# zz990099/foundationpose_cpp

Measured on AMD Instinct MI355X. Metric: pose-hypotheses/sec (Register N=252, 640x480), higher is better.
Workload: dtype f16; 1 GPU; Register N=252 hypotheses, 640x480 refine_itr=1, frame resident in HBM; mesh=synthetic ellipsoid V=2562 F=5120, 512x512 texture, weights=synthetic (seed 7), precision=f16 storage / f32 accumulate (the reference's TensorRT --fp16), parallelism=single GPU, collective=none

## Files before the change

foundationpose_cpp_amd/csrc/fp_geometry.hip:

```cpp

#include "fp_internal.h"
#include <cstdlib>

namespace fp {

#define CR_SUBPIXEL_LOG2 4
#define CR_MAXVIEWPORT_LOG2 11
#define CR_DEPTH_MIN (2200u << 3)
#define CR_DEPTH_MAX (0xFFFFFFFFu - (2200u << 3))

static constexpr int CROP = FP_CROP_HW;

struct K9 { float k[9]; };

__device__ __forceinline__ float clampf(float f, float a, float b) { return fmaxf(a, fminf(f, b)); }

template <bool FMAD> __device__ __forceinline__ float mad(float a, float b, float c) { return FMAD ? fmaf(a, b, c) : a * b + c; }
template <bool FMAD> __device__ __forceinline__ float dot3(float a0, float b0, float a1, float b1, float a2, float b2) {
  return mad<FMAD>(a2, b2, mad<FMAD>(a1, b1, a0 * b0));
}
template <bool FMAD> __device__ __forceinline__ float diffprod(float a, float b, float c, float d) {
  return FMAD ? fmaf(a, b, -(c * d)) : a * b - c * d;
}

// ... 378 lines not shown
    }
    if (!culled) {
      out = TRI_ROWS_ALL;
      if ((v0.w >= fabsf(v0.z)) & (v1.w >= fabsf(v1.z)) & (v2.w >= fabsf(v2.z))) {
        const float vs = (float)(CROP << (CR_SUBPIXEL_LOG2 - 1));
        const float rw0 = 1.0f / v0.w, rw1 = 1.0f / v1.w, rw2 = 1.0f / v2.w;
        const int ax = f32_to_s32_sat(v0.x * rw0 * vs), ay = f32_to_s32_sat(v0.y * rw0 * vs);
        const int bx_ = f32_to_s32_sat(v1.x * rw1 * vs), by_ = f32_to_s32_sat(v1.y * rw1 * vs);
        const int cx = f32_to_s32_sat(v2.x * rw2 * vs), cy = f32_to_s32_sat(v2.y * rw2 * vs);
        const int loxy = min(imin3(ax, bx_, cx), imin3(ay, by_, cy));
        const int hixy = max(imax3(ax, bx_, cx), imax3(ay, by_, cy));
        const int aabbLimit = (1 << (CR_MAXVIEWPORT_LOG2 + CR_SUBPIXEL_LOG2)) - 1;
        if (loxy >= -32768 && hixy <= 32767 && hixy - loxy <= aabbLimit) {
          const int area = (bx_ - ax) * (cy - ay) - (by_ - ay) * (cx - ax);
          const int bx = (CROP - 1) << (CR_SUBPIXEL_LOG2 - 1);
          const int px0 = max((imin3(ax, bx_, cx) + bx + 15) >> 4, 0), px1 = min((imax3(ax, bx_, cx) + bx) >> 4, CROP - 1);
          const int py0 = max((imin3(ay, by_, cy) + bx + 15) >> 4, 0), py1 = min((imax3(ay, by_, cy) + bx) >> 4, CROP - 1);
          out = (area == 0 || px0 > px1 || py0 > py1) ? TRI_ROWS_EMPTY : ((unsigned)py0 | ((unsigned)py1 << 16));
        }
      }
    }
  }
  return out;
}
__global__ __launch_bounds__(256) void tri_rows_kernel(const int32_t *__restrict__ faces, int F, int V, const float4 *__restrict__ clip_all,
                                                       unsigned *__restrict__ rows_all) {
  const int f = blockIdx.x * 256 + threadIdx.x, n = blockIdx.y;
  if (f >= F) return;
  const float4 *clip = clip_all + (size_t)n * V;
  unsigned out = TRI_ROWS_EMPTY;
  const int i0 = faces[f * 3], i1 = faces[f * 3 + 1], i2 = faces[f * 3 + 2];
  if ((unsigned)i0 < (unsigned)V && (unsigned)i1 < (unsigned)V && (unsigned)i2 < (unsigned)V) out = tri_rows_of(clip[i0], clip[i1], clip[i2]);
  rows_all[(size_t)n * F + f] = out;
}
void launch_tri_rows(hipStream_t s, const DeviceMesh &m, int N, const float4 *clip, unsigned *rows) {
  if (m.F <= 0 || N <= 0) return;
  hipLaunchKernelGGL(tri_rows_kernel, dim3((m.F + 255) / 256, N), dim3(256), 0, s, m.faces, m.F, m.V, clip, rows);
}
constexpr int TRI_LIST = 8192;

template <int MODE, int STRIP_ROWS, int NT, bool FMAD, bool VCOL = false>
__global__ __launch_bounds__(NT) void raster_shade_kernel(
    const int32_t *__restrict__ faces, int F, int V, const float *__restrict__ uvs, const uint8_t *__restrict__ tex,
    int TH, int TW, float downscale, const PoseRec *__restrict__ recs, const float4 *__restrict__ clip_all,
    const float4 *__restrict__ attr_all, void *__restrict__ out_all, int32_t *__restrict__ tri_id_dbg,
    float *__restrict__ rast_dbg, const unsigned *__restrict__ tri_rows_all, const uint32_t *__restrict__ vcol = nullptr) {
  extern __shared__ __attribute__((aligned(16))) unsigned char smem[];
  unsigned long long *zbuf = reinterpret_cast<unsigned long long *>(smem);
  const int strip = blockIdx.x, n = blockIdx.y, tid = threadIdx.x;
  const int row0 = strip * STRIP_ROWS;
  const float4 *clip = clip_all + (size_t)n * V;
  const float4 *attr = attr_all + (size_t)n * V;

  const unsigned long long clear_key = ((unsigned long long)CR_DEPTH_MAX << 32) | 0xFFFFFFFFull;
  for (int i = tid; i < STRIP_ROWS * CROP; i += NT) zbuf[i] = clear_key;
  __syncthreads();

  auto process = [&](int f, const float4 &v0, const float4 &v1, const float4 &v2) {
    if ((v0.w < fabsf(v0.x)) | (v0.w < fabsf(v0.y)) | (v0.w < fabsf(v0.z))) {
      if (((v0.w < +v0.x) & (v1.w < +v1.x) & (v2.w < +v2.x)) | ((v0.w < -v0.x) & (v1.w < -v1.x) & (v2.w < -v2.x)) |
          ((v0.w < +v0.y) & (v1.w < +v1.y) & (v2.w < +v2.y)) | ((v0.w < -v0.y) & (v1.w < -v1.y) & (v2.w < -v2.y)) |
          ((v0.w < +v0.z) & (v1.w < +v1.z) & (v2.w < +v2.z)) | ((v0.w < -v0.z) & (v1.w < -v1.z) & (v2.w < -v2.z)))
        return;
    }
    bool fast = false;
    if ((v0.w >= fabsf(v0.z)) & (v1.w >= fabsf(v1.z)) & (v2.w >= fabsf(v2.z))) {
      const float vs = (float)(CROP << (CR_SUBPIXEL_LOG2 - 1));
      float rw0 = 1.0f / v0.w, rw1 = 1.0f / v1.w, rw2 = 1.0f / v2.w;
      int ax = f32_to_s32_sat(v0.x * rw0 * vs), ay = f32_to_s32_sat(v0.y * rw0 * vs);
      int bx_ = f32_to_s32_sat(v1.x * rw1 * vs), by_ = f32_to_s32_sat(v1.y * rw1 * vs);
      int cx = f32_to_s32_sat(v2.x * rw2 * vs), cy = f32_to_s32_sat(v2.y * rw2 * vs);
      int loxy = min(imin3(ax, bx_, cx), imin3(ay, by_, cy));
      int hixy = max(imax3(ax, bx_, cx), imax3(ay, by_, cy));
      const int aabbLimit = (1 << (CR_MAXVIEWPORT_LOG2 + CR_SUBPIXEL_LOG2)) - 1;
      fast = (loxy >= -32768 && hixy <= 32767 && hixy - loxy <= aabbLimit);
    }
    if (fast) raster_one<STRIP_ROWS>(v0, v1, v2, (unsigned)(f + 1), row0, zbuf);
    else raster_clipped<STRIP_ROWS, FMAD>(v0, v1, v2, (unsigned)(f + 1), row0, zbuf);
  };
  struct Tri { int i0, i1, i2; };
  auto load_idx = [&](int f) {
    Tri t{-1, -1, -1};
    if (f < F) { t.i0 = faces[f * 3]; t.i1 = faces[f * 3 + 1]; t.i2 = faces[f * 3 + 2]; }
    return t;
  };
  auto valid = [&](const Tri &t) { return (unsigned)t.i0 < (unsigned)V && (unsigned)t.i1 < (unsigned)V && (unsigned)t.i2 < (unsigned)V; };
  const float4 zero4 = make_float4(0.f, 0.f, 0.f, 0.f);
  if (tri_rows_all) {
    static_assert(TRI_LIST >= 8 * NT, "a slab of 4 NT triangles must fit behind the flush threshold");
    unsigned *list = reinterpret_cast<unsigned *>(zbuf + STRIP_ROWS * CROP);
    unsigned *count = list + TRI_LIST;
    const unsigned *tri_rows = tri_rows_all + (size_t)n * F;
    const unsigned row_last = (unsigned)(row0 + STRIP_ROWS - 1);
    if (tid == 0) *count = 0u;
    __syncthreads();
    auto flush = [&]() {
      const int nl = (int)*count;
      auto entry = [&](int k) { return k < nl ? load_idx((int)list[k]) : Tri{-1, -1, -1}; };
      Tri cur = entry(tid), nxt = entry(tid + NT);
      bool ok = valid(cur);
      float4 v0 = ok ? clip[cur.i0] : zero4, v1 = ok ? clip[cur.i1] : zero4, v2 = ok ? clip[cur.i2] : zero4;
      for (int k = tid; k < nl; k += NT) {
        const bool okn = valid(nxt);
        const float4 w0 = okn ? clip[nxt.i0] : zero4, w1 = okn ? clip[nxt.i1] : zero4, w2 = okn ? clip[nxt.i2] : zero4;
        const Tri nn = entry(k + 2 * NT);
        if (ok) process((int)list[k], v0, v1, v2);
        v0 = w0; v1 = w1; v2 = w2; ok = okn; nxt = nn;
      }
    };
    auto load_slab = [&](int base, unsigned (&r)[4]) {
#pragma unroll
      for (int u = 0; u < 4; u++) {
        const int f = base + u * NT + tid;
        r[u] = f < F ? tri_rows[f] : TRI_ROWS_EMPTY;
      }
    };
    unsigned r[4], rn[4];
    load_slab(0, r);
    for (int base = 0; base < F; base += 4 * NT) {
      load_slab(base + 4 * NT, rn);
#pragma unroll
      for (int u = 0; u < 4; u++)
        if ((r[u] & 0xffffu) <= row_last && (r[u] >> 16) >= (unsigned)row0) list[atomicAdd(count, 1u)] = (unsigned)(base + u * NT + tid);
      __syncthreads();
      const bool full = *count > (unsigned)(TRI_LIST - 4 * NT) && base + 4 * NT < F;
      __syncthreads();
      if (full) {
        flush();
        __syncthreads();
        if (tid == 0) *count = 0u;
        __syncthreads();
      }
#pragma unroll
      for (int u = 0; u < 4; u++) r[u] = rn[u];
    }
    flush();
  } else {
    Tri cur = load_idx(tid), nxt = load_idx(tid + NT);
    bool ok = valid(cur);
    float4 v0 = ok ? clip[cur.i0] : zero4, v1 = ok ? clip[cur.i1] : zero4, v2 = ok ? clip[cur.i2] : zero4;
    for (int f = tid; f < F; f += NT) {
      const bool okn = valid(nxt);
      const float4 w0 = okn ? clip[nxt.i0] : zero4, w1 = okn ? clip[nxt.i1] : zero4, w2 = okn ? clip[nxt.i2] : zero4;
      const Tri nn = load_idx(f + 2 * NT);
      if (ok) process(f, v0, v1, v2);
      v0 = w0; v1 = w1; v2 = w2; ok = okn; nxt = nn;
    }
  }
  __syncthreads();

  const PoseRec &rec = recs[n];
  const float tpx = rec.pose[12], tpy = rec.pose[13], tpz = rec.pose[14];
  const float xs = 2.f / (float)CROP, xo = 1.f / (float)CROP - 1.f;
  for (int i = tid; i < STRIP_ROWS * CROP; i += NT) {
    int ly = i / CROP, px = i - ly * CROP, py = row0 + ly;
    unsigned color = ~(unsigned)(zbuf[i] & 0xFFFFFFFFull);
    int triIdx = (int)color - 1;
    float b0 = 0, b1 = 0, zw = 0, idf = 0;
    float xyz0 = 0, xyz1 = 0, xyz2 = 0, uu = 0, vv = 0, dif = 0;
    float vc[3] = {0, 0, 0};
    if (triIdx >= 0 && triIdx < F) {
      int vi0 = faces[triIdx * 3], vi1 = faces[triIdx * 3 + 1], vi2 = faces[triIdx * 3 + 2];
      float4 p0 = clip[vi0], p1 = clip[vi1], p2 = clip[vi2];
      float fx = mad<FMAD>(xs, (float)px, xo), fy = mad<FMAD>(xs, (float)py, xo);
      float p0x = mad<FMAD>(-fx, p0.w, p0.x), p0y = mad<FMAD>(-fy, p0.w, p0.y);
      float p1x = mad<FMAD>(-fx, p1.w, p1.x), p1y = mad<FMAD>(-fy, p1.w, p1.y);
      float p2x = mad<FMAD>(-fx, p2.w, p2.x), p2y = mad<FMAD>(-fy, p2.w, p2.y);
      float a0 = diffprod<FMAD>(p1x, p2y, p1y, p2x), a1 = diffprod<FMAD>(p2x, p0y, p2y, p0x), a2 = diffprod<FMAD>(p0x, p1y, p0y, p1x);
      float iw = 1.f / (a0 + a1 + a2);
      b0 = a0 * iw; b1 = a1 * iw;
      float z = dot3<FMAD>(p0.z, a0, p1.z, a1, p2.z, a2), w = dot3<FMAD>(p0.w, a0, p1.w, a1, p2.w, a2);
      zw = z / w;
      b0 = clampf(b0, 0.f, 1.f); b1 = clampf(b1, 0.f, 1.f);
      if (b0 != b0) b0 = 0.f;
      if (b1 != b1) b1 = 0.f;
      zw = fmaxf(fminf(zw, 1.f), -1.f);
      idf = (float)(triIdx + 1);
      float b2 = 1.f - b0 - b1;
      float4 q0 = attr[vi0], q1 = attr[vi1], q2 = attr[vi2];
      xyz0 = dot3<FMAD>(b0, q0.x, b1, q1.x, b2, q2.x);
      xyz1 = dot3<FMAD>(b0, q0.y, b1, q1.y, b2, q2.y);
      xyz2 = dot3<FMAD>(b0, q0.z, b1, q1.z, b2, q2.z);
      dif = dot3<FMAD>(b0, q0.w, b1, q1.w, b2, q2.w);
      if constexpr (VCOL) {
        const uint32_t c0 = vcol[vi0], c1 = vcol[vi1], c2 = vcol[vi2];
        const float sc = 1.0f / 255.0f;
#pragma unroll
        for (int c = 0; c < 3; c++)
          vc[c] = dot3<FMAD>(b0, (float)((c0 >> (8 * c)) & 255u) * sc, b1, (float)((c1 >> (8 * c)) & 255u) * sc, b2,
                             (float)((c2 >> (8 * c)) & 255u) * sc);
      } else {
        uu = dot3<FMAD>(b0, uvs[vi0 * 2], b1, uvs[vi1 * 2], b2, uvs[vi2 * 2]);
        vv = dot3<FMAD>(b0, uvs[vi0 * 2 + 1], b1, uvs[vi1 * 2 + 1], b2, uvs[vi2 * 2 + 1]);
      }
    }
    if (tri_id_dbg) tri_id_dbg[((size_t)n * CROP + py) * CROP + px] = (int)color;
    if (rast_dbg) {
      float *ro = rast_dbg + (((size_t)n * CROP + py) * CROP + px) * 4;
      ro[0] = b0; ro[1] = b1; ro[2] = zw; ro[3] = idf;
    }
    float o[6];
    float fg = clampf(idf, 0, 1);
    if (VCOL && fg > 0.0f) {
      const float shade = mad<FMAD>(dif, 0.5f, 0.8f);
      for (int c = 0; c < 3; c++) o[c] = clampf(vc[c] * shade * fg, 0.0f, 1.0f);
    } else if (!VCOL && fg > 0.0f) {
      float u = uu - floorf(uu), v = vv - floorf(vv);
      u = mad<FMAD>(u, (float)TW, -0.5f); v = mad<FMAD>(v, (float)TH, -0.5f);
      int iu0 = (int)floorf(u), iv0 = (int)floorf(v);
      int iu1 = iu0 + 1, iv1 = iv0 + 1;
      u -= (float)iu0; v -= (float)iv0;
      if (iu0 < 0) iu0 += TW;
      if (iv0 < 0) iv0 += TH;
      if (iu1 >= TW) iu1 -= TW;
      if (iv1 >= TH) iv1 -= TH;
      const float sc = 1.0f / 255.0f;
      const uint8_t *t00 = tex + (iu0 + TW * iv0) * 3, *t10 = tex + (iu1 + TW * iv0) * 3;
      const uint8_t *t01 = tex + (iu0 + TW * iv1) * 3, *t11 = tex + (iu1 + TW * iv1) * 3;
      float shade = mad<FMAD>(dif, 0.5f, 0.8f);
      for (int c = 0; c < 3; c++) {
        float a00 = (float)t00[c] * sc, a10 = (float)t10[c] * sc, a01 = (float)t01[c] * sc, a11 = (float)t11[c] * sc;
        float top = mad<FMAD>(u, a10 - a00, a00), bot = mad<FMAD>(u, a11 - a01, a01);
        float rgb = mad<FMAD>(v, bot - top, top);
        float q = rgb * shade * fg;
        o[c] = clampf(clampf(q, 0, 1), 0.0f, 1.0f);
      }
    } else {
      o[0] = o[1] = o[2] = 0.0f;
    }
    {
      bool invalid = xyz2 < FP_MIN_DEPTH;
      float q0 = (xyz0 - tpx) / downscale, q1 = (xyz1 - tpy) / downscale, q2 = (xyz2 - tpz) / downscale;
      o[3] = (fabsf(q0) > FP_MAX_DEPTH || invalid) ? 0.0f : q0;
      o[4] = (fabsf(q1) > FP_MAX_DEPTH || invalid) ? 0.0f : q1;
      o[5] = (fabsf(q2) > FP_MAX_DEPTH || invalid) ? 0.0f : q2;
    }
    size_t opix = ((size_t)n * CROP + (CROP - 1 - py)) * CROP + px;
    if (MODE == OUT_F32X6) {
      float *d = reinterpret_cast<float *>(out_all) + opix * 6;
      float2 *d2 = reinterpret_cast<float2 *>(d);
      d2[0] = make_float2(o[0], o[1]); d2[1] = make_float2(o[2], o[3]); d2[2] = make_float2(o[4], o[5]);
    } else {
      reinterpret_cast<uint4 *>(out_all)[s2d_index((size_t)n, CROP - 1 - py, px)] = pack6<MODE>(o);
    }
  }
}

static thread_local const unsigned *t_tri_rows = nullptr;
static size_t tri_list_lds() { return t_tri_rows ? (size_t)TRI_LIST * 4 + 16 : 0; }

#ifdef FP_TEST_HOOKS
static int g_tri_rows_tall = 0;
void set_tri_rows_tall(int v) { g_tri_rows_tall = v; }
#else
static constexpr int g_tri_rows_tall = 0;
#endif
#ifdef FP_TEST_HOOKS
static int g_strip_threads = 0;
void set_raster_strip_threads(int t) { g_strip_threads = t; }
#else
static constexpr int g_strip_threads = 0;
#endif

template <int MODE, int STRIP_ROWS, bool FMAD, bool VCOL>
static void launch_raster_shade_t(hipStream_t s, const DeviceMesh &m, const PoseRec *recs, int N, const float4 *clip,
                                  const float4 *attr, void *out, int32_t *tri_id_dbg, float *rast_dbg) {
  size_t lds = (size_t)STRIP_ROWS * CROP * sizeof(unsigned long long) + tri_list_lds();
  dim3 grid(CROP / STRIP_ROWS, N), block(256);
  float downscale = m.diameter / 2;
  if constexpr (STRIP_ROWS == 8 && MODE != OUT_F32X6) if (!tri_id_dbg && !rast_dbg && g_strip_threads != 256) {
    if (g_strip_threads == 1024 || (g_strip_threads == 0 && N <= 25)) {
      hipLaunchKernelGGL((raster_shade_kernel<MODE, STRIP_ROWS, 1024, FMAD, VCOL>), grid, dim3(1024), lds, s, m.faces, m.F, m.V, m.uvs,
                         m.tex, m.TH, m.TW, downscale, recs, clip, attr, out, tri_id_dbg, rast_dbg, t_tri_rows, m.vcol);
      return;
    }
    if (g_strip_threads == 512 || (g_strip_threads == 0 && N < 48)) {
      hipLaunchKernelGGL((raster_shade_kernel<MODE, STRIP_ROWS, 512, FMAD, VCOL>), grid, dim3(512), lds, s, m.faces, m.F, m.V, m.uvs,
                         m.tex, m.TH, m.TW, downscale, recs, clip, attr, out, tri_id_dbg, rast_dbg, t_tri_rows, m.vcol);
      return;
    }
  }
  if constexpr (STRIP_ROWS >= 40) {
    static PerDeviceOnce attr_once;
    attr_once.run([] {
      (void)hipFuncSetAttribute((const void *)raster_shade_kernel<MODE, STRIP_ROWS, 256, FMAD, VCOL>, hipFuncAttributeMaxDynamicSharedMemorySize,
                                (int)((size_t)STRIP_ROWS * CROP * sizeof(unsigned long long) + (size_t)TRI_LIST * 4 + 16));
    });
  }
  hipLaunchKernelGGL((raster_shade_kernel<MODE, STRIP_ROWS, 256, FMAD, VCOL>), grid, block, lds, s, m.faces, m.F, m.V, m.uvs, m.tex,
                     m.TH, m.TW, downscale, recs, clip, attr, out, tri_id_dbg, rast_dbg, t_tri_rows, m.vcol);
}

#ifdef FP_TEST_HOOKS
static int g_strip_rows_override = 0;
void set_raster_strip_rows(int r) { g_strip_rows_override = r; }
#else
static constexpr int g_strip_rows_override = 0;
#endif

template <int MODE, int STRIP_ROWS, bool FMAD, bool VCOL>
static void launch_raster_tall(hipStream_t s, const DeviceMesh &m, const PoseRec *recs, int N, const float4 *clip,
                               const float4 *attr, void *out) {
  const size_t lds_max = (size_t)STRIP_ROWS * CROP * sizeof(unsigned long long) + (size_t)TRI_LIST * 4 + 16;
  size_t lds = (size_t)STRIP_ROWS * CROP * sizeof(unsigned long long) + tri_list_lds();
  static PerDeviceOnce attr_once;
  attr_once.run([lds_max] {
    (void)hipFuncSetAttribute((const void *)raster_shade_kernel<MODE, STRIP_ROWS, 1024, FMAD, VCOL>, hipFuncAttributeMaxDynamicSharedMemorySize,
                              (int)lds_max);
  });
  hipLaunchKernelGGL((raster_shade_kernel<MODE, STRIP_ROWS, 1024, FMAD, VCOL>), dim3(CROP / STRIP_ROWS, N), dim3(1024), lds, s, m.faces, m.F,
                     m.V, m.uvs, m.tex, m.TH, m.TW, m.diameter / 2, recs, clip, attr, out, nullptr, nullptr, t_tri_rows, m.vcol);
}

static int strip_rows_for(int N) { return g_strip_rows_override ? g_strip_rows_override : (N >= 100 ? 1080 : (N >= 48 ? 20 : 8)); }
bool raster_wants_tri_rows(int N) { return strip_rows_for(N) < 1000 || g_tri_rows_tall; }

template <int MODE, bool FMAD, bool VCOL>
static void launch_raster_mode(hipStream_t s, const DeviceMesh &m, const PoseRec *recs, int N, const float4 *clip,
                               const float4 *attr, void *out, int32_t *tri_id_dbg, float *rast_dbg) {
  int rows = strip_rows_for(N);
  if constexpr (MODE != OUT_F32X6) if (rows > 1000 && !tri_id_dbg && !rast_dbg) {
    if (rows == 1080) { launch_raster_tall<MODE, 80, FMAD, VCOL>(s, m, recs, N, clip, attr, out); return; }
#ifdef FP_TEST_HOOKS
    if (rows == 1040) launch_raster_tall<MODE, 40, FMAD, VCOL>(s, m, recs, N, clip, attr, out);
    else launch_raster_tall<MODE, 20, FMAD, VCOL>(s, m, recs, N, clip, attr, out);
    return;
#endif
  }
  if (rows > 1000) rows = 20;
#ifdef FP_TEST_HOOKS
  if (rows == 40) { launch_raster_shade_t<MODE, 40, FMAD, VCOL>(s, m, recs, N, clip, attr, out, tri_id_dbg, rast_dbg); return; }
#endif
  if (rows == 20) { launch_raster_shade_t<MODE, 20, FMAD, VCOL>(s, m, recs, N, clip, attr, out, tri_id_dbg, rast_dbg); return; }
  if constexpr (MODE != OUT_F32X6) if ((rows == 4 || (rows == 8 && N <= 2 && !g_strip_rows_override)) && !tri_id_dbg && !rast_dbg) {
    const size_t lds = (size_t)4 * CROP * sizeof(unsigned long long) + tri_list_lds();
    hipLaunchKernelGGL((raster_shade_kernel<MODE, 4, 1024, FMAD, VCOL>), dim3(CROP / 4, N), dim3(1024), lds, s, m.faces, m.F, m.V, m.uvs,
                       m.tex, m.TH, m.TW, m.diameter / 2, recs, clip, attr, out, tri_id_dbg, rast_dbg, t_tri_rows, m.vcol);
    return;
  }
  launch_raster_shade_t<MODE, 8, FMAD, VCOL>(s, m, recs, N, clip, attr, out, tri_id_dbg, rast_dbg);
}

void launch_raster_shade(hipStream_t s, const DeviceMesh &m, const PoseRec *recs, int N, const float4 *clip,
                         const float4 *attr, OutMode mode, void *out, int32_t *tri_id_dbg, float *rast_dbg, bool fmad,
                         const unsigned *tri_rows) {
  t_tri_rows = tri_rows;
#define FP_RASTER_MODE(MODE)                                                                                      \
  do {                                                                                                            \
    if (m.vcol) {                                                                                                 \
      if (fmad) launch_raster_mode<MODE, true, true>(s, m, recs, N, clip, attr, out, tri_id_dbg, rast_dbg);       \
      else launch_raster_mode<MODE, false, true>(s, m, recs, N, clip, attr, out, tri_id_dbg, rast_dbg);           \
    } else if (fmad) launch_raster_mode<MODE, true, false>(s, m, recs, N, clip, attr, out, tri_id_dbg, rast_dbg); \
    else launch_raster_mode<MODE, false, false>(s, m, recs, N, clip, attr, out, tri_id_dbg, rast_dbg);            \
  } while (0)
  if (mode == OUT_F32X6) FP_RASTER_MODE(OUT_F32X6);
  else if (mode == OUT_BF16X8) FP_RASTER_MODE(OUT_BF16X8);
  else FP_RASTER_MODE(OUT_F16X8);
#undef FP_RASTER_MODE
}

__global__ __launch_bounds__(256) void sampler_scan_kernel(const float *__restrict__ depth, const uint8_t *__restrict__ mask,
                                                           int H, int W, float min_depth, int *__restrict__ state,
                                                           float *__restrict__ vals) {
  const int i = blockIdx.x * 256 + threadIdx.x;
  const bool in = i < H * W;
  const bool m = in && mask[i] > 0;
  const int v = in ? i / W : 0, u = in ? i - v * W : 0;
  if (__any(m)) {
    int umin = m ? u : 0x7fffffff, umax = m ? u : -1, vmin = m ? v : 0x7fffffff, vmax = m ? v : -1;
#pragma unroll
    for (int o = 32; o > 0; o >>= 1) {
      umin = min(umin, __shfl_xor(umin, o)); umax = max(umax, __shfl_xor(umax, o));
      vmin = min(vmin, __shfl_xor(vmin, o)); vmax = max(vmax, __shfl_xor(vmax, o));
    }
    if ((threadIdx.x & 63) == 0) {
      atomicMin(&state[0], umin); atomicMax(&state[1], umax);
      atomicMin(&state[2], vmin); atomicMax(&state[3], vmax);
    }
  }
  const float d = m ? depth[i] : 0.f;
  const bool valid = m && d >= min_depth;
  const unsigned long long ball = __ballot(valid);
  if (ball) {
    const int lane = threadIdx.x & 63;
    int base = 0;
    if (lane == 0) base = atomicAdd(&state[4], __popcll(ball));
    base = __shfl(base, 0);
    if (valid) vals[base + __popcll(ball & ((1ull << lane) - 1ull))] = d;
  }
}

__device__ unsigned radix_select(const unsigned *keys, int n, int k, unsigned *hist , unsigned *sh ) {
  unsigned prefix = 0, pmask = 0;
  for (int pass = 3; pass >= 0; pass--) {
    for (int b = threadIdx.x; b < 256; b += blockDim.x) hist[b] = 0;
    __syncthreads();
    const int shift = pass * 8;
    for (int i = threadIdx.x; i < n; i += blockDim.x) {
      unsigned key = keys[i];
      if ((key & pmask) == prefix) atomicAdd(&hist[(key >> shift) & 255], 1u);
    }
    __syncthreads();
    if (threadIdx.x == 0) {
      unsigned acc = 0, b = 0;
      for (; b < 256; b++) {
        if (acc + hist[b] > (unsigned)k) break;
        acc += hist[b];
      }
      sh[0] = b; sh[1] = acc;
    }
    __syncthreads();
    prefix |= sh[0] << shift;
    pmask |= 255u << shift;
    k -= (int)sh[1];
    __syncthreads();
  }
  return prefix;
}

__global__ __launch_bounds__(1024) void sampler_pose_kernel(int *__restrict__ state, const float *__restrict__ vals, K9 K,
                                                            const float *__restrict__ grid, int first, int N,
                                                            float *__restrict__ poses) {
  __shared__ unsigned hist[256];
  __shared__ unsigned sh[2];
  __shared__ float center[3];
  const int n = state[4];
  const int umin = state[0], umax = state[1], vmin = state[2], vmax = state[3];
  const bool bad = umax < 0 || n <= 0;
  const unsigned *keys = reinterpret_cast<const unsigned *>(vals);
  unsigned hi_bits = 0, lo_bits = 0;
  if (!bad) {
    hi_bits = radix_select(keys, n, n / 2, hist, sh);
    lo_bits = hi_bits;
    if ((n & 1) == 0) lo_bits = radix_select(keys, n, n / 2 - 1, hist, sh);
  }
  __syncthreads();
  if (threadIdx.x == 0) {
    state[0] = 0x7fffffff; state[1] = -1; state[2] = 0x7fffffff; state[3] = -1; state[4] = 0;
    state[6] = bad ? (umax < 0 ? 1 : 2) : 0;
  }
  if (bad) return;
  if (threadIdx.x == 0) {
    const float hi = __uint_as_float(hi_bits), lo = __uint_as_float(lo_bits);
    const float zc = (n & 1) ? hi : (float)(((double)lo + (double)hi) / 2.0);
    const float uc = (float)((umin + umax) / 2.0), vc = (float)((vmin + vmax) / 2.0);
    const float *m = K.k;
    float c00 = m[4] * m[8] - m[5] * m[7], c01 = m[5] * m[6] - m[3] * m[8], c02 = m[3] * m[7] - m[4] * m[6];
    float det = m[0] * c00 + m[1] * c01 + m[2] * c02, id = 1.0f / det;
    float Ki[9] = {c00 * id, (m[2] * m[7] - m[1] * m[8]) * id, (m[1] * m[5] - m[2] * m[4]) * id,
                   c01 * id, (m[0] * m[8] - m[2] * m[6]) * id, (m[2] * m[3] - m[0] * m[5]) * id,
                   c02 * id, (m[1] * m[6] - m[0] * m[7]) * id, (m[0] * m[4] - m[1] * m[3]) * id};
    for (int r = 0; r < 3; r++) {
      float sacc = Ki[r * 3] * uc;
      sacc = sacc + Ki[r * 3 + 1] * vc;
      sacc = sacc + Ki[r * 3 + 2] * 1.0f;
      center[r] = sacc * zc;
    }
  }
  __syncthreads();
  for (int i = threadIdx.x; i < N * 16; i += blockDim.x) {
    const int e = i & 15;
    poses[i] = (e >= 12 && e < 15) ? center[e - 12] : grid[(size_t)first * 16 + i];
  }
}

void launch_sampler(hipStream_t s, const float *filtered_depth, const uint8_t *mask_dev, int H, int W, float min_depth,
                    const float *K9_host, const float *grid_dev, int first, int N, int *state, float *vals, float *poses) {
  hipLaunchKernelGGL(sampler_scan_kernel, dim3((H * W + 255) / 256), dim3(256), 0, s, filtered_depth, mask_dev, H, W, min_depth,
                     state, vals);
  K9 K;
  for (int i = 0; i < 9; i++) K.k[i] = K9_host[i];
  hipLaunchKernelGGL(sampler_pose_kernel, dim3(1), dim3(1024), 0, s, state, vals, K, grid_dev, first, N, poses);
}


template <int MODE>
__device__ __forceinline__ void crop_body(const FrameRef *__restrict__ frame, int H, int W, float fx, float fy, float cx, float cy,
                                          const PoseRec &rec, float downscale, void *__restrict__ out_all, int n, int i) {
  const uint8_t *__restrict__ rgb = frame->rgb;
  const float *__restrict__ depth = frame->depth;
  const int P = frame->pitch > 0 ? frame->pitch : W;
  const int wx0 = frame->wx0, wy0 = frame->wy0, wx1 = frame->wx1, wy1 = frame->wy1;
  const int y = i / CROP, x = i - y * CROP;
  float sxf = rec.m0 * (float)x + rec.m2, syf = rec.m4 * (float)y + rec.m5;
  sxf = fminf(fmaxf(sxf, -16777216.0f), 16777216.0f);
  syf = fminf(fmaxf(syf, -16777216.0f), 16777216.0f);
  float o[6];
  {
    int x0 = (int)floorf(sxf), y0 = (int)floorf(syf);
    float ax = sxf - (float)x0, ay = syf - (float)y0;
    bool vx0 = x0 >= 0 && x0 < W && x0 >= wx0 && x0 < wx1, vx1 = x0 + 1 >= 0 && x0 + 1 < W && x0 + 1 >= wx0 && x0 + 1 < wx1;
    bool vy0 = y0 >= 0 && y0 < H && y0 >= wy0 && y0 < wy1, vy1 = y0 + 1 >= 0 && y0 + 1 < H && y0 + 1 >= wy0 && y0 + 1 < wy1;
    const uint8_t *r0 = rgb + ((long long)y0 * P + x0) * 3, *r1 = rgb + ((long long)(y0 + 1) * P + x0) * 3;
    float w00 = (1.0f - ax) * (1.0f - ay), w10 = ax * (1.0f - ay), w01 = (1.0f - ax) * ay, w11 = ax * ay;
    for (int ch = 0; ch < 3; ch++) {
      float p00 = (vy0 && vx0) ? (float)r0[ch] : 0.0f, p10 = (vy0 && vx1) ? (float)r0[3 + ch] : 0.0f;
      float p01 = (vy1 && vx0) ? (float)r1[ch] : 0.0f, p11 = (vy1 && vx1) ? (float)r1[3 + ch] : 0.0f;
      float val = p00 * w00 + p10 * w10 + p01 * w01 + p11 * w11;
      float q = rintf(val);
      q = q < 0 ? 0 : (q > 255 ? 255 : q);
      o[ch] = q * (1.0f / 255.0f);
    }
  }
  {
    int xn = (int)floorf(sxf + 0.5f), yn = (int)floorf(syf + 0.5f);
    float p0 = 0, p1 = 0, p2 = 0;
    if (xn >= 0 && xn < W && yn >= 0 && yn < H && xn >= wx0 && xn < wx1 && yn >= wy0 && yn < wy1) {
      float d = depth[(long long)yn * P + xn];
      if (!(d < 0.001f)) { p0 = ((float)xn - cx) * d / fx; p1 = ((float)yn - cy) * d / fy; p2 = d; }
    }
    bool invalid = p2 < FP_MIN_DEPTH;
    float q0 = (p0 - rec.pose[12]) / downscale, q1 = (p1 - rec.pose[13]) / downscale, q2 = (p2 - rec.pose[14]) / downscale;
    o[3] = (fabsf(q0) > FP_MAX_DEPTH || invalid) ? 0.0f : q0;
    o[4] = (fabsf(q1) > FP_MAX_DEPTH || invalid) ? 0.0f : q1;
    o[5] = (fabsf(q2) > FP_MAX_DEPTH || invalid) ? 0.0f : q2;
  }
  size_t opix = (size_t)n * CROP * CROP + i;
  if (MODE == OUT_F32X6) {
    float2 *d2 = reinterpret_cast<float2 *>(reinterpret_cast<float *>(out_all) + opix * 6);
    d2[0] = make_float2(o[0], o[1]); d2[1] = make_float2(o[2], o[3]); d2[2] = make_float2(o[4], o[5]);
  } else {
    reinterpret_cast<uint4 *>(out_all)[s2d_index((size_t)n, y, x)] = pack6<MODE>(o);
  }
}

template <int MODE>
__global__ __launch_bounds__(256) void crop_kernel(const FrameRef *__restrict__ frame,
                                                   int H, int W, float fx, float fy, float cx, float cy,
                                                   const PoseRec *__restrict__ recs, float downscale,
                                                   void *__restrict__ out_all) {
  const int n = blockIdx.y;
  const int i = blockIdx.x * 256 + threadIdx.x;
  if (i >= CROP * CROP) return;
  crop_body<MODE>(frame, H, W, fx, fy, cx, cy, recs[n], downscale, out_all, n, i);
}

template <bool FMAD, int MODE>
__global__ __launch_bounds__(256) void vertex_crop_kernel(const float *__restrict__ verts, const float *__restrict__ normals, int V, int nvb,
                                                          PoseRec *__restrict__ recs, float4 *__restrict__ clip, float4 *__restrict__ attr,
                                                          const PoseSetupArgs sa, const FrameRef *__restrict__ frame, int n_crop,
                                                          void *__restrict__ out_b, const int32_t *__restrict__ faces, int F,
                                                          unsigned *__restrict__ tri_rows) {
  const int n = blockIdx.y;
  PoseRec own;
  constexpr int NCB = (CROP * CROP + 255) / 256;
  if ((int)blockIdx.x >= nvb + NCB) {
    const int f = ((int)blockIdx.x - nvb - NCB) * 256 + threadIdx.x;
    if (f >= F) return;
    unsigned out = TRI_ROWS_EMPTY;
    const int i0 = faces[f * 3], i1 = faces[f * 3 + 1], i2 = faces[f * 3 + 2];
    if ((unsigned)i0 < (unsigned)V && (unsigned)i1 < (unsigned)V && (unsigned)i2 < (unsigned)V) {
      make_pose_rec(sa.poses, n, sa.K, sa.img_h, sa.img_w, sa.crop_ratio, sa.diameter, own);
      const float4 c0 = clip_of<FMAD>(own, verts[i0 * 3], verts[i0 * 3 + 1], verts[i0 * 3 + 2]);
      const float4 c1 = clip_of<FMAD>(own, verts[i1 * 3], verts[i1 * 3 + 1], verts[i1 * 3 + 2]);
      const float4 c2 = clip_of<FMAD>(own, verts[i2 * 3], verts[i2 * 3 + 1], verts[i2 * 3 + 2]);
      out = tri_rows_of(c0, c1, c2);
    }
    tri_rows[(size_t)n * F + f] = out;
    return;
  }
  if ((int)blockIdx.x < nvb) {
    const int v = blockIdx.x * 256 + threadIdx.x;
    if (v >= V) return;
    make_pose_rec(sa.poses, n, sa.K, sa.img_h, sa.img_w, sa.crop_ratio, sa.diameter, own);
    if (v == 0) recs[n] = own;
    vertex_body<FMAD>(verts, normals, V, v, n, own, clip, attr, nullptr, 0ull);
    return;
  }
  const int i = ((int)blockIdx.x - nvb) * 256 + threadIdx.x;
  if (n >= n_crop || i >= CROP * CROP) return;
  make_pose_rec(sa.poses, n, sa.K, sa.img_h, sa.img_w, sa.crop_ratio, sa.diameter, own);
  crop_body<MODE>(frame, sa.img_h, sa.img_w, sa.K.k[0], sa.K.k[4], sa.K.k[2], sa.K.k[5], own, sa.diameter / 2, out_b, n, i);
}

bool launch_setup_vertex_crop(hipStream_t s, const DeviceMesh &m, const float *poses_dev, int N, const float *K9_host, int img_h, int img_w,
                              float crop_ratio, float diameter, PoseRec *recs, float4 *clip, float4 *attr, bool fmad, const FrameRef *frame,
                              int n_crop, OutMode mode, void *out_b, unsigned *tri_rows) {
  if (mode == OUT_F32X6) return false;
  PoseSetupArgs sa;
  sa.poses = poses_dev;
  for (int i = 0; i < 9; i++) sa.K.k[i] = K9_host[i];
  sa.img_h = img_h; sa.img_w = img_w; sa.crop_ratio = crop_ratio; sa.diameter = diameter;
  const int nvb = (m.V + 255) / 256;
  const int ntb = tri_rows && m.F > 0 ? (m.F + 255) / 256 : 0;
  const dim3 grid(nvb + (CROP * CROP + 255) / 256 + ntb, N);
#define FP_VC(FM_, MD_) hipLaunchKernelGGL((vertex_crop_kernel<FM_, MD_>), grid, dim3(256), 0, s, m.verts, m.normals, m.V, nvb, recs, clip, attr, sa, frame, n_crop, out_b, m.faces, m.F, tri_rows)
  if (mode == OUT_BF16X8) { if (fmad) FP_VC(true, OUT_BF16X8); else FP_VC(false, OUT_BF16X8); }
  else { if (fmad) FP_VC(true, OUT_F16X8); else FP_VC(false, OUT_F16X8); }
#undef FP_VC
  return true;
}

void launch_crop(hipStream_t s, const FrameRef *frame, int H, int W, const float *K, const PoseRec *recs,
                 int N, float diameter, OutMode mode, void *out) {
  dim3 grid((CROP * CROP + 255) / 256, N), block(256);
  float downscale = diameter / 2;
  if (mode == OUT_F32X6)
    hipLaunchKernelGGL(crop_kernel<OUT_F32X6>, grid, block, 0, s, frame, H, W, K[0], K[4], K[2], K[5], recs,
                       downscale, out);
  else if (mode == OUT_BF16X8)
    hipLaunchKernelGGL(crop_kernel<OUT_BF16X8>, grid, block, 0, s, frame, H, W, K[0], K[4], K[2], K[5], recs,
                       downscale, out);
  else
    hipLaunchKernelGGL(crop_kernel<OUT_F16X8>, grid, block, 0, s, frame, H, W, K[0], K[4], K[2], K[5], recs,
                       downscale, out);
}


__global__ void depth_to_xyz_kernel(const float *__restrict__ depth, int H, int W, float fx, float fy, float cx,
                                    float cy, float *__restrict__ xyz) {
  int p = blockIdx.x * blockDim.x + threadIdx.x;
  if (p >= H * W) return;
  int r = p / W, c = p - r * W;
  float d = depth[p];
  float x = 0, y = 0, z = 0;
  if (!(d < 0.001f)) { x = ((float)c - cx) * d / fx; y = ((float)r - cy) * d / fy; z = d; }
  xyz[(size_t)p * 3] = x; xyz[(size_t)p * 3 + 1] = y; xyz[(size_t)p * 3 + 2] = z;
}

__global__ __launch_bounds__(256) void window_fetch_kernel(const uint4 *__restrict__ src_host, uint4 *__restrict__ dst, unsigned n16) {
  for (unsigned i = blockIdx.x * 256 + threadIdx.x; i < n16; i += gridDim.x * 256) dst[i] = src_host[i];
}
void launch_window_fetch(hipStream_t s, const void *src_host_mapped, void *dst, size_t bytes) {
  const unsigned n16 = (unsigned)((bytes + 15) / 16);
  const unsigned blocks = std::min(256u, (n16 + 255) / 256);
  hipLaunchKernelGGL(window_fetch_kernel, dim3(blocks), dim3(256), 0, s, (const uint4 *)src_host_mapped, (uint4 *)dst, n16);
}

void launch_depth_to_xyz(hipStream_t s, const float *depth, int H, int W, const float *K, float *xyz) {
  hipLaunchKernelGGL(depth_to_xyz_kernel, dim3((H * W + 255) / 256), dim3(256), 0, s, depth, H, W, K[0], K[4], K[2],
                     K[5], xyz);
}

__global__ void erode_kernel(const float *__restrict__ depth, float *__restrict__ out, int H, int W) {
  const int radius = 2;
  const float depth_diff_thres = 0.001f, ratio_thres = 0.8f, zfar = 100.0f;
  int w = blockIdx.x * blockDim.x + threadIdx.x, h = blockIdx.y * blockDim.y + threadIdx.y;
  if (w >= W || h >= H) return;
  float d_ori = depth[h * W + w];
  if (d_ori < 0.1f || d_ori >= zfar) { out[h * W + w] = 0.0f; return; }
  float bad = 0.0f, total = 0.0f;
  for (int u = w - radius; u <= w + radius; u++) {
    if (u < 0 || u >= W) continue;
    for (int v = h - radius; v <= h + radius; v++) {
      if (v < 0 || v >= H) continue;
      float cur = depth[v * W + u];
      total += 1.0f;
      if (cur < 0.1f || cur >= zfar || fabsf(cur - d_ori) > depth_diff_thres) bad += 1.0f;
    }
  }
  out[h * W + w] = ((bad / total) > ratio_thres) ? 0.0f : d_ori;
}

__global__ void bilateral_kernel(const float *__restrict__ depth, float *__restrict__ out, int H, int W) {
  const int radius = 2;
  const float zfar = 100.0f, sigmaD = 2.0f, sigmaR = 100000.0f;
  int w = blockIdx.x * blockDim.x + threadIdx.x, h = blockIdx.y * blockDim.y + threadIdx.y;
  if (w >= W || h >= H) return;
  float mean = 0.0f;
  int nvalid = 0;
  for (int u = w - radius; u <= w + radius; u++) {
    if (u < 0 || u >= W) continue;
    for (int v = h - radius; v <= h + radius; v++) {
      if (v < 0 || v >= H) continue;
      float cur = depth[v * W + u];
      if (cur >= 0.1f && cur < zfar) { nvalid++; mean += cur; }
    }
  }
  if (nvalid == 0) { out[h * W + w] = 0.0f; return; }
  mean /= (float)nvalid;
  float dc = depth[h * W + w], sw = 0.0f, sum = 0.0f;
// ... 161 lines not shown
```

Baseline: 23860 hypotheses/s.

## Batch shading gathers, remap pixels to 2x2 quads, merge median radix selects

The raster shading pass now handles two pixels per thread. It issues all vertex, attribute, uv and texel gathers before the arithmetic and skips them when no pixel in the wave hits a triangle. For packed output modes, the shading and crop kernels walk pixels in 2x2 quad order so the space-to-depth stores land contiguously. The depth-median sampler runs the two order statistics for an even count in one radix pass sequence, using wave-aggregated histogram atomics and a shuffle-based prefix scan. The cost is higher register pressure and more index arithmetic.

New measurement: 23890 hypotheses/s (median of 6 runs). About the same (+0.1%).

```diff
diff --git a/foundationpose_cpp_amd/csrc/fp_geometry.hip b/foundationpose_cpp_amd/csrc/fp_geometry.hip
--- a/foundationpose_cpp_amd/csrc/fp_geometry.hip
+++ b/foundationpose_cpp_amd/csrc/fp_geometry.hip
@@ -554,96 +554,164 @@
   const PoseRec &rec = recs[n];
   const float tpx = rec.pose[12], tpy = rec.pose[13], tpz = rec.pose[14];
   const float xs = 2.f / (float)CROP, xo = 1.f / (float)CROP - 1.f;
-  for (int i = tid; i < STRIP_ROWS * CROP; i += NT) {
-    int ly = i / CROP, px = i - ly * CROP, py = row0 + ly;
-    unsigned color = ~(unsigned)(zbuf[i] & 0xFFFFFFFFull);
-    int triIdx = (int)color - 1;
-    float b0 = 0, b1 = 0, zw = 0, idf = 0;
-    float xyz0 = 0, xyz1 = 0, xyz2 = 0, uu = 0, vv = 0, dif = 0;
-    float vc[3] = {0, 0, 0};
-    if (triIdx >= 0 && triIdx < F) {
-      int vi0 = faces[triIdx * 3], vi1 = faces[triIdx * 3 + 1], vi2 = faces[triIdx * 3 + 2];
-      float4 p0 = clip[vi0], p1 = clip[vi1], p2 = clip[vi2];
-      float fx = mad<FMAD>(xs, (float)px, xo), fy = mad<FMAD>(xs, (float)py, xo);
-      float p0x = mad<FMAD>(-fx, p0.w, p0.x), p0y = mad<FMAD>(-fy, p0.w, p0.y);
-      float p1x = mad<FMAD>(-fx, p1.w, p1.x), p1y = mad<FMAD>(-fy, p1.w, p1.y);
-      float p2x = mad<FMAD>(-fx, p2.w, p2.x), p2y = mad<FMAD>(-fy, p2.w, p2.y);
-      float a0 = diffprod<FMAD>(p1x, p2y, p1y, p2x), a1 = diffprod<FMAD>(p2x, p0y, p2y, p0x), a2 = diffprod<FMAD>(p0x, p1y, p0y, p1x);
-      float iw = 1.f / (a0 + a1 + a2);
-      b0 = a0 * iw; b1 = a1 * iw;
-      float z = dot3<FMAD>(p0.z, a0, p1.z, a1, p2.z, a2), w = dot3<FMAD>(p0.w, a0, p1.w, a1, p2.w, a2);
-      zw = z / w;
-      b0 = clampf(b0, 0.f, 1.f); b1 = clampf(b1, 0.f, 1.f);
-      if (b0 != b0) b0 = 0.f;
-      if (b1 != b1) b1 = 0.f;
-      zw = fmaxf(fminf(zw, 1.f), -1.f);
-      idf = (float)(triIdx + 1);
-      float b2 = 1.f - b0 - b1;
-      float4 q0 = attr[vi0], q1 = attr[vi1], q2 = attr[vi2];
-      xyz0 = dot3<FMAD>(b0, q0.x, b1, q1.x, b2, q2.x);
-      xyz1 = dot3<FMAD>(b0, q0.y, b1, q1.y, b2, q2.y);
-      xyz2 = dot3<FMAD>(b0, q0.z, b1, q1.z, b2, q2.z);
-      dif = dot3<FMAD>(b0, q0.w, b1, q1.w, b2, q2.w);
-      if constexpr (VCOL) {
-        const uint32_t c0 = vcol[vi0], c1 = vcol[vi1], c2 = vcol[vi2];
+  constexpr int NPIX = STRIP_ROWS * CROP;
+  constexpr int SHADE_U = NPIX > NT ? 2 : 1;
+  static_assert(STRIP_ROWS % 2 == 0, "the shading pass walks row pairs");
+  for (int base = 0; base < NPIX; base += SHADE_U * NT) {
+    int px[SHADE_U], py[SHADE_U];
+    unsigned color[SHADE_U];
+    bool live[SHADE_U], hit[SHADE_U];
+    bool any_hit = false;
+#pragma unroll
+    for (int u = 0; u < SHADE_U; u++) {
+      const int i = base + u * NT + tid;
+      live[u] = i < NPIX;
+      const int pair = i / (2 * CROP), q = i - pair * (2 * CROP);
+      const int ly = MODE == OUT_F32X6 ? i / CROP : pair * 2 + ((q >> 1) & 1);
+      px[u] = MODE == OUT_F32X6 ? i - ly * CROP : (q >> 2) * 2 + (q & 1);
+      py[u] = row0 + ly;
+      color[u] = live[u] ? ~(unsigned)(zbuf[ly * CROP + px[u]] & 0xFFFFFFFFull) : 0u;
+      const int triIdx = (int)color[u] - 1;
+      hit[u] = triIdx >= 0 && triIdx < F;
+      any_hit |= hit[u];
+    }
+    float b0[SHADE_U], b1[SHADE_U], zw[SHADE_U], idf[SHADE_U];
+    float xyz0[SHADE_U], xyz1[SHADE_U], xyz2[SHADE_U], uu[SHADE_U], vv[SHADE_U], dif[SHADE_U];
+    float vc[SHADE_U][3];
+#pragma unroll
+    for (int u = 0; u < SHADE_U; u++) {
+      b0[u] = b1[u] = zw[u] = idf[u] = 0; xyz0[u] = xyz1[u] = xyz2[u] = uu[u] = vv[u] = dif[u] = 0;
+      vc[u][0] = vc[u][1] = vc[u][2] = 0;
+    }
+    const bool wave_hit = __any(any_hit);
+    if (wave_hit) {
+      int vi0[SHADE_U], vi1[SHADE_U], vi2[SHADE_U];
+#pragma unroll
+      for (int u = 0; u < SHADE_U; u++) {
+        const int t3 = hit[u] ? ((int)color[u] - 1) * 3 : 0;
+        vi0[u] = faces[t3]; vi1[u] = faces[t3 + 1]; vi2[u] = faces[t3 + 2];
+      }
+#pragma unroll
+      for (int u = 0; u < SHADE_U; u++)
+        if (!hit[u]) vi0[u] = vi1[u] = vi2[u] = 0;
+      float4 p0[SHADE_U], p1[SHADE_U], p2[SHADE_U], q0[SHADE_U], q1[SHADE_U], q2[SHADE_U];
+      float tu0[SHADE_U], tu1[SHADE_U], tu2[SHADE_U], tv0[SHADE_U], tv1[SHADE_U], tv2[SHADE_U];
+      uint32_t c0[SHADE_U], c1[SHADE_U], c2[SHADE_U];
+#pragma unroll
+      for (int u = 0; u < SHADE_U; u++) {
+        p0[u] = clip[vi0[u]]; p1[u] = clip[vi1[u]]; p2[u] = clip[vi2[u]];
+        q0[u] = attr[vi0[u]]; q1[u] = attr[vi1[u]]; q2[u] = attr[vi2[u]];
+        if constexpr (VCOL) {
+          c0[u] = vcol[vi0[u]]; c1[u] = vcol[vi1[u]]; c2[u] = vcol[vi2[u]];
+        } else {
+          tu0[u] = uvs[vi0[u] * 2]; tu1[u] = uvs[vi1[u] * 2]; tu2[u] = uvs[vi2[u] * 2];
+          tv0[u] = uvs[vi0[u] * 2 + 1]; tv1[u] = uvs[vi1[u] * 2 + 1]; tv2[u] = uvs[vi2[u] * 2 + 1];
+        }
+      }
+#pragma unroll
+      for (int u = 0; u < SHADE_U; u++) {
+        if (!hit[u]) continue;
+        const int triIdx = (int)color[u] - 1;
+        float fx = mad<FMAD>(xs, (float)px[u], xo), fy = mad<FMAD>(xs, (float)py[u], xo);
+        float p0x = mad<FMAD>(-fx, p0[u].w, p0[u].x), p0y = mad<FMAD>(-fy, p0[u].w, p0[u].y);
+        float p1x = mad<FMAD>(-fx, p1[u].w, p1[u].x), p1y = mad<FMAD>(-fy, p1[u].w, p1[u].y);
+        float p2x = mad<FMAD>(-fx, p2[u].w, p2[u].x), p2y = mad<FMAD>(-fy, p2[u].w, p2[u].y);
+        float a0 = diffprod<FMAD>(p1x, p2y, p1y, p2x), a1 = diffprod<FMAD>(p2x, p0y, p2y, p0x), a2 = diffprod<FMAD>(p0x, p1y, p0y, p1x);
+        float iw = 1.f / (a0 + a1 + a2);
+        float c0b = a0 * iw, c1b = a1 * iw;
+        float z = dot3<FMAD>(p0[u].z, a0, p1[u].z, a1, p2[u].z, a2), w = dot3<FMAD>(p0[u].w, a0, p1[u].w, a1, p2[u].w, a2);
+        float zwv = z / w;
+        c0b = clampf(c0b, 0.f, 1.f); c1b = clampf(c1b, 0.f, 1.f);
+        if (c0b != c0b) c0b = 0.f;
+        if (c1b != c1b) c1b = 0.f;
+        zwv = fmaxf(fminf(zwv, 1.f), -1.f);
+        b0[u] = c0b; b1[u] = c1b; zw[u] = zwv;
+        idf[u] = (float)(triIdx + 1);
+        float b2 = 1.f - c0b - c1b;
+        xyz0[u] = dot3<FMAD>(c0b, q0[u].x, c1b, q1[u].x, b2, q2[u].x);
+        xyz1[u] = dot3<FMAD>(c0b, q0[u].y, c1b, q1[u].y, b2, q2[u].y);
+        xyz2[u] = dot3<FMAD>(c0b, q0[u].z, c1b, q1[u].z, b2, q2[u].z);
+        dif[u] = dot3<FMAD>(c0b, q0[u].w, c1b, q1[u].w, b2, q2[u].w);
+        if constexpr (VCOL) {
+          const float sc = 1.0f / 255.0f;
+#pragma unroll
+          for (int c = 0; c < 3; c++)
+            vc[u][c] = dot3<FMAD>(c0b, (float)((c0[u] >> (8 * c)) & 255u) * sc, c1b, (float)((c1[u] >> (8 * c)) & 255u) * sc, b2,
+                                  (float)((c2[u] >> (8 * c)) & 255u) * sc);
+        } else {
+          uu[u] = dot3<FMAD>(c0b, tu0[u], c1b, tu1[u], b2, tu2[u]);
+          vv[u] = dot3<FMAD>(c0b, tv0[u], c1b, tv1[u], b2, tv2[u]);
+        }
+      }
+    }
+    float fg[SHADE_U], tfu[SHADE_U], tfv[SHADE_U];
+    uint8_t tx[SHADE_U][4][3];
+#pragma unroll
+    for (int u = 0; u < SHADE_U; u++) {
+      fg[u] = clampf(idf[u], 0, 1);
+      tfu[u] = tfv[u] = 0.f;
+      for (int k = 0; k < 4; k++) for (int c = 0; c < 3; c++) tx[u][k][c] = 0;
+    }
+    if constexpr (!VCOL) if (wave_hit) {
+#pragma unroll
+      for (int u = 0; u < SHADE_U; u++) {
+        const bool lit = fg[u] > 0.0f;
+        float tu = uu[u] - floorf(uu[u]), tv = vv[u] - floorf(vv[u]);
+        tu = mad<FMAD>(tu, (float)TW, -0.5f); tv = mad<FMAD>(tv, (float)TH, -0.5f);
+        int iu0 = (int)floorf(tu), iv0 = (int)floorf(tv);
+        int iu1 = iu0 + 1, iv1 = iv0 + 1;
+        tu -= (float)iu0; tv -= (float)iv0;
+        if (iu0 < 0) iu0 += TW;
+        if (iv0 < 0) iv0 += TH;
+        if (iu1 >= TW) iu1 -= TW;
+        if (iv1 >= TH) iv1 -= TH;
+        tfu[u] = tu; tfv[u] = tv;
+        const uint8_t *t00 = tex + (lit ? (iu0 + TW * iv0) * 3 : 0), *t10 = tex + (lit ? (iu1 + TW * iv0) * 3 : 0);
+        const uint8_t *t01 = tex + (lit ? (iu0 + TW * iv1) * 3 : 0), *t11 = tex + (lit ? (iu1 + TW * iv1) * 3 : 0);
+#pragma unroll
+        for (int c = 0; c < 3; c++) { tx[u][0][c] = t00[c]; tx[u][1][c] = t10[c]; tx[u][2][c] = t01[c]; tx[u][3][c] = t11[c]; }
+      }
+    }
+#pragma unroll
+    for (int u = 0; u < SHADE_U; u++) {
+      if (!live[u]) continue;
+      if (tri_id_dbg) tri_id_dbg[((size_t)n * CROP + py[u]) * CROP + px[u]] = (int)color[u];
+      if (rast_dbg) {
+        float *ro = rast_dbg + (((size_t)n * CROP + py[u]) * CROP + px[u]) * 4;
+        ro[0] = b0[u]; ro[1] = b1[u]; ro[2] = zw[u]; ro[3] = idf[u];
+      }
+      float o[6];
+      if (VCOL && fg[u] > 0.0f) {
+        const float shade = mad<FMAD>(dif[u], 0.5f, 0.8f);
+        for (int c = 0; c < 3; c++) o[c] = clampf(vc[u][c] * shade * fg[u], 0.0f, 1.0f);
+      } else if (!VCOL && fg[u] > 0.0f) {
         const float sc = 1.0f / 255.0f;
-#pragma unroll
-        for (int c = 0; c < 3; c++)
-          vc[c] = dot3<FMAD>(b0, (float)((c0 >> (8 * c)) & 255u) * sc, b1, (float)((c1 >> (8 * c)) & 255u) * sc, b2,
-                             (float)((c2 >> (8 * c)) & 255u) * sc);
+        float shade = mad<FMAD>(dif[u], 0.5f, 0.8f);
+        for (int c = 0; c < 3; c++) {
+          float a00 = (float)tx[u][0][c] * sc, a10 = (float)tx[u][1][c] * sc, a01 = (float)tx[u][2][c] * sc, a11 = (float)tx[u][3][c] * sc;
+          float top = mad<FMAD>(tfu[u], a10 - a00, a00), bot = mad<FMAD>(tfu[u], a11 - a01, a01);
+          float rgb = mad<FMAD>(tfv[u], bot - top, top);
+          float q = rgb * shade * fg[u];
+          o[c] = clampf(clampf(q, 0, 1), 0.0f, 1.0f);
+        }
       } else {
-        uu = dot3<FMAD>(b0, uvs[vi0 * 2], b1, uvs[vi1 * 2], b2, uvs[vi2 * 2]);
-        vv = dot3<FMAD>(b0, uvs[vi0 * 2 + 1], b1, uvs[vi1 * 2 + 1], b2, uvs[vi2 * 2 + 1]);
-      }
-    }
-    if (tri_id_dbg) tri_id_dbg[((size_t)n * CROP + py) * CROP + px] = (int)color;
-    if (rast_dbg) {
-      float *ro = rast_dbg + (((size_t)n * CROP + py) * CROP + px) * 4;
-      ro[0] = b0; ro[1] = b1; ro[2] = zw; ro[3] = idf;
-    }
-    float o[6];
-    float fg = clampf(idf, 0, 1);
-    if (VCOL && fg > 0.0f) {
-      const float shade = mad<FMAD>(dif, 0.5f, 0.8f);
-      for (int c = 0; c < 3; c++) o[c] = clampf(vc[c] * shade * fg, 0.0f, 1.0f);
-    } else if (!VCOL && fg > 0.0f) {
-      float u = uu - floorf(uu), v = vv - floorf(vv);
-      u = mad<FMAD>(u, (float)TW, -0.5f); v = mad<FMAD>(v, (float)TH, -0.5f);
-      int iu0 = (int)floorf(u), iv0 = (int)floorf(v);
-      int iu1 = iu0 + 1, iv1 = iv0 + 1;
-      u -= (float)iu0; v -= (float)iv0;
-      if (iu0 < 0) iu0 += TW;
-      if (iv0 < 0) iv0 += TH;
-      if (iu1 >= TW) iu1 -= TW;
-      if (iv1 >= TH) iv1 -= TH;
-      const float sc = 1.0f / 255.0f;
-      const uint8_t *t00 = tex + (iu0 + TW * iv0) * 3, *t10 = tex + (iu1 + TW * iv0) * 3;
-      const uint8_t *t01 = tex + (iu0 + TW * iv1) * 3, *t11 = tex + (iu1 + TW * iv1) * 3;
-      float shade = mad<FMAD>(dif, 0.5f, 0.8f);
-      for (int c = 0; c < 3; c++) {
-        float a00 = (float)t00[c] * sc, a10 = (float)t10[c] * sc, a01 = (float)t01[c] * sc, a11 = (float)t11[c] * sc;
-        float top = mad<FMAD>(u, a10 - a00, a00), bot = mad<FMAD>(u, a11 - a01, a01);
-        float rgb = mad<FMAD>(v, bot - top, top);
-        float q = rgb * shade * fg;
-        o[c] = clampf(clampf(q, 0, 1), 0.0f, 1.0f);
-      }
-    } else {
-      o[0] = o[1] = o[2] = 0.0f;
-    }
-    {
-      bool invalid = xyz2 < FP_MIN_DEPTH;
-      float q0 = (xyz0 - tpx) / downscale, q1 = (xyz1 - tpy) / downscale, q2 = (xyz2 - tpz) / downscale;
-      o[3] = (fabsf(q0) > FP_MAX_DEPTH || invalid) ? 0.0f : q0;
-      o[4] = (fabsf(q1) > FP_MAX_DEPTH || invalid) ? 0.0f : q1;
-      o[5] = (fabsf(q2) > FP_MAX_DEPTH || invalid) ? 0.0f : q2;
-    }
-    size_t opix = ((size_t)n * CROP + (CROP - 1 - py)) * CROP + px;
-    if (MODE == OUT_F32X6) {
-      float *d = reinterpret_cast<float *>(out_all) + opix * 6;
-      float2 *d2 = reinterpret_cast<float2 *>(d);
-      d2[0] = make_float2(o[0], o[1]); d2[1] = make_float2(o[2], o[3]); d2[2] = make_float2(o[4], o[5]);
-    } else {
-      reinterpret_cast<uint4 *>(out_all)[s2d_index((size_t)n, CROP - 1 - py, px)] = pack6<MODE>(o);
+        o[0] = o[1] = o[2] = 0.0f;
+      }
+      {
+        bool invalid = xyz2[u] < FP_MIN_DEPTH;
+        float q0 = (xyz0[u] - tpx) / downscale, q1 = (xyz1[u] - tpy) / downscale, q2 = (xyz2[u] - tpz) / downscale;
+        o[3] = (fabsf(q0) > FP_MAX_DEPTH || invalid) ? 0.0f : q0;
+        o[4] = (fabsf(q1) > FP_MAX_DEPTH || invalid) ? 0.0f : q1;
+        o[5] = (fabsf(q2) > FP_MAX_DEPTH || invalid) ? 0.0f : q2;
+      }
+      size_t opix = ((size_t)n * CROP + (CROP - 1 - py[u])) * CROP + px[u];
+      if (MODE == OUT_F32X6) {
+        float *d = reinterpret_cast<float *>(out_all) + opix * 6;
+        float2 *d2 = reinterpret_cast<float2 *>(d);
+        d2[0] = make_float2(o[0], o[1]); d2[1] = make_float2(o[2], o[3]); d2[2] = make_float2(o[4], o[5]);
+      } else {
+        reinterpret_cast<uint4 *>(out_all)[s2d_index((size_t)n, CROP - 1 - py[u], px[u])] = pack6<MODE>(o);
+      }
     }
   }
 }
@@ -792,39 +860,82 @@
   }
 }
 
-__device__ unsigned radix_select(const unsigned *keys, int n, int k, unsigned *hist , unsigned *sh ) {
-  unsigned prefix = 0, pmask = 0;
+__device__ __forceinline__ void count_digit(unsigned *h, unsigned d, bool m) {
+  const int lane = threadIdx.x & 63;
+  unsigned long long todo = __ballot(m);
+#pragma unroll 1
+  for (int round = 0; round < 4 && todo; round++) {
+    const int leader = __ffsll((long long)todo) - 1;
+    const unsigned dl = (unsigned)__builtin_amdgcn_readlane((int)d, leader);
+    const unsigned long long same = __ballot(m && d == dl);
+    if (lane == leader) atomicAdd(&h[dl], (unsigned)__popcll(same));
+    m = m && d != dl;
+    todo &= ~same;
+  }
+  if (m) atomicAdd(&h[d], 1u);
+}
+
+struct Select2 { unsigned a, b; };
+__device__ Select2 radix_select2(const unsigned *__restrict__ keys, int n, unsigned ka, unsigned kb, bool two, unsigned (*hist)[256] ,
+                                 unsigned *sh ) {
+  const int tid = threadIdx.x, lane = tid & 63, wave = tid >> 6, nt = blockDim.x;
+  unsigned pa = 0, pb = 0, pmask = 0;
+  bool split = false;
   for (int pass = 3; pass >= 0; pass--) {
-    for (int b = threadIdx.x; b < 256; b += blockDim.x) hist[b] = 0;
+    for (int b = tid; b < 512; b += nt) (&hist[0][0])[b] = 0;
     __syncthreads();
     const int shift = pass * 8;
-    for (int i = threadIdx.x; i < n; i += blockDim.x) {
-      unsigned key = keys[i];
-      if ((key & pmask) == prefix) atomicAdd(&hist[(key >> shift) & 255], 1u);
+    for (int base = 0; base < n; base += 4 * nt) {
+      unsigned key[4];
+      bool in[4];
+#pragma unroll
+      for (int u = 0; u < 4; u++) {
+        const int i = base + u * nt + tid;
+        in[u] = i < n;
+        key[u] = in[u] ? keys[i] : 0u;
+      }
+#pragma unroll
+      for (int u = 0; u < 4; u++) {
+        const unsigned d = (key[u] >> shift) & 255u, up = key[u] & pmask;
+        count_digit(hist[0], d, in[u] && up == pa);
+        if (split) count_digit(hist[1], d, in[u] && up == pb);
+      }
     }
     __syncthreads();
-    if (threadIdx.x == 0) {
-      unsigned acc = 0, b = 0;
-      for (; b < 256; b++) {
-        if (acc + hist[b] > (unsigned)k) break;
-        acc += hist[b];
-      }
-      sh[0] = b; sh[1] = acc;
+    if (wave == 0 || (wave == 1 && two)) {
+      const unsigned *h = hist[split ? wave : 0];
+      const unsigned k = wave ? kb : ka;
+      const unsigned h0 = h[lane * 4], h1 = h[lane * 4 + 1], h2 = h[lane * 4 + 2], h3 = h[lane * 4 + 3];
+      const unsigned own = h0 + h1 + h2 + h3;
+      unsigned incl = own;
+#pragma unroll
+      for (int o = 1; o < 64; o <<= 1) {
+        const unsigned t = __shfl_up(incl, o);
+        if (lane >= o) incl += t;
+      }
+      unsigned c = incl - own;
+      const unsigned hh[4] = {h0, h1, h2, h3};
+#pragma unroll
+      for (int j = 0; j < 4; j++) {
+        if (c <= k && k < c + hh[j]) { sh[wave * 2] = (unsigned)(lane * 4 + j); sh[wave * 2 + 1] = c; }
+        c += hh[j];
+      }
     }
     __syncthreads();
-    prefix |= sh[0] << shift;
+    const unsigned ba = sh[0], ca = sh[1], bb = two ? sh[2] : ba, cb = two ? sh[3] : ca;
+    pa |= ba << shift; ka -= ca;
+    pb |= bb << shift; kb -= cb;
+    split = split || ba != bb;
     pmask |= 255u << shift;
-    k -= (int)sh[1];
-    __syncthreads();
-  }
-  return prefix;
+  }
+  return Select2{pa, pb};
 }
 
 __global__ __launch_bounds__(1024) void sampler_pose_kernel(int *__restrict__ state, const float *__restrict__ vals, K9 K,
                                                             const float *__restrict__ grid, int first, int N,
                                                             float *__restrict__ poses) {
-  __shared__ unsigned hist[256];
-  __shared__ unsigned sh[2];
+  __shared__ unsigned hist[2][256];
+  __shared__ unsigned sh[4];
   __shared__ float center[3];
   const int n = state[4];
   const int umin = state[0], umax = state[1], vmin = state[2], vmax = state[3];
@@ -832,9 +943,10 @@
   const unsigned *keys = reinterpret_cast<const unsigned *>(vals);
   unsigned hi_bits = 0, lo_bits = 0;
   if (!bad) {
-    hi_bits = radix_select(keys, n, n / 2, hist, sh);
-    lo_bits = hi_bits;
-    if ((n & 1) == 0) lo_bits = radix_select(keys, n, n / 2 - 1, hist, sh);
+    const bool two = (n & 1) == 0;
+    const Select2 sel = radix_select2(keys, n, (unsigned)(n / 2), two ? (unsigned)(n / 2 - 1) : (unsigned)(n / 2), two, hist, sh);
+    hi_bits = sel.a;
+    lo_bits = two ? sel.b : sel.a;
   }
   __syncthreads();
   if (threadIdx.x == 0) {
@@ -883,7 +995,9 @@
   const float *__restrict__ depth = frame->depth;
   const int P = frame->pitch > 0 ? frame->pitch : W;
   const int wx0 = frame->wx0, wy0 = frame->wy0, wx1 = frame->wx1, wy1 = frame->wy1;
-  const int y = i / CROP, x = i - y * CROP;
+  const int pair = i / (2 * CROP), qd = i - pair * (2 * CROP);
+  const int y = MODE == OUT_F32X6 ? i / CROP : pair * 2 + ((qd >> 1) & 1);
+  const int x = MODE == OUT_F32X6 ? i - y * CROP : (qd >> 2) * 2 + (qd & 1);
   float sxf = rec.m0 * (float)x + rec.m2, syf = rec.m4 * (float)y + rec.m5;
   sxf = fminf(fmaxf(sxf, -16777216.0f), 16777216.0f);
   syf = fminf(fmaxf(syf, -16777216.0f), 16777216.0f);
@@ -917,8 +1031,8 @@
     o[4] = (fabsf(q1) > FP_MAX_DEPTH || invalid) ? 0.0f : q1;
     o[5] = (fabsf(q2) > FP_MAX_DEPTH || invalid) ? 0.0f : q2;
   }
-  size_t opix = (size_t)n * CROP * CROP + i;
   if (MODE == OUT_F32X6) {
+    size_t opix = (size_t)n * CROP * CROP + i;
     float2 *d2 = reinterpret_cast<float2 *>(reinterpret_cast<float *>(out_all) + opix * 6);
     d2[0] = make_float2(o[0], o[1]); d2[1] = make_float2(o[2], o[3]); d2[2] = make_float2(o[4], o[5]);
   } else {
```
